# daooshee/ReReVST-Code

Measured on AMD Instinct MI355X. Metric: stylized frames/sec at 512x512, 1 style, higher is better.
Workload: dtype f32

## Files before the change

rerevst-code_amd/csrc/rerevst_hip.hip:

```cpp
#include <hip/hip_runtime.h>
#include <dlfcn.h>
#include <stddef.h>
#include <stdint.h>
#include <string.h>
#include <algorithm>
#include <cmath>
#include <thread>
#include <stdio.h>
#include <map>
#include <condition_variable>
#include <mutex>
#include <string>
#include <vector>

#include "../../include/rerevst_hip.h"
#include "conv_mfma.h"
#include "conv_wino.h"
#include "conv_wino_split.h"
#include "conv_f43.h"
#include "conv_thin.h"
#include "prep_kernels.h"
#include "mask_kernels.h"

namespace {

const int NORM_CH[11] = {512, 512, 256, 128, 64, 256, 256, 128, 128, 64, 64};
enum { N_DEC0 = 0, N_DEC1, N_DEC2, N_DEC3, N_DEC4, N_S4N1, N_S4N2, N_S3N1, N_S3N2, N_S2N1, N_S2N2 };
const int STYLE_CH[4] = {64, 128, 256, 512};
// ... 154 lines not shown
    unsigned launch_gen = 0;
    struct Feature { float* p; int H, W; uint8_t* u8; bool owned = true; };
    std::vector<Feature> features;
    std::vector<void*> feat_blocks;
    size_t feat_cap = (size_t)64 << 30, feat_bytes = 0;
    std::vector<float*> patches;
    int patch_h = 0, patch_w = 0, add_H = 0, add_W = 0;
    uint8_t* d_u8 = nullptr; size_t d_u8_cap = 0;
    float* d_outf = nullptr; size_t d_outf_cap = 0;
    double *stat_part = nullptr, *stat_part2 = nullptr, *stat_acc = nullptr;
    float *stat_mean = nullptr, *prep_cmean = nullptr;
    size_t ws_cap = (size_t)64 << 30;
    int last_groups = 0, last_group_size = 0; size_t last_ws_bytes = 0;
    PrepPlan prep;
    uint8_t* pend_u8 = nullptr; size_t pend_cap = 0; int pend_n = 0;
    InFmt pend_in = IN_BGR8;
    static constexpr int BLEND_W_RING = 4, BLEND_W_FLOATS = 64 * RRV_MAX_STYLES;
    struct BlendW { float* dev = nullptr; float* pin = nullptr; hipEvent_t ev[BLEND_W_RING] = {nullptr}; bool used[BLEND_W_RING] = {false}; unsigned gen = 0; } blend_w[2];
    const float* last_pre = nullptr; int last_pre_H = 0, last_pre_W = 0, last_pre_B = 0;
    struct StageBufs { uint8_t* in = nullptr; void* out = nullptr; size_t in_cap = 0, out_cap = 0; };
    struct HostStage {
        StageBufs dev, pin; hipEvent_t in_done = nullptr, k_done = nullptr, out_done = nullptr;
        float *mask = nullptr, *mask_pin = nullptr; size_t mask_cap = 0, mask_pin_cap = 0;
    } hstage[4];
    hipStream_t copy_in = nullptr, copy_out = nullptr;
    struct Ticket { long id = -1; void* out = nullptr; size_t out_bytes = 0; bool open = false; } tickets[4];
    long next_ticket = 0;
    int grid_share = 1;
    int f43_mode = 1;
    unsigned f43_layers = F43_DEFAULT_LAYERS;
    bool illcond = false;
    bool enc_p8_tables = false;
    int p8 = 3;
    bool f43_path = false;
    unsigned direct_layers = 0;
    int ms_group = 0;
    YuvSide yuv_in, yuv_out;
    int host_io = 0;
    int n_cus = 256;
    int debug = 0;
    int fail_alloc_in = 0;
    bool profiling = false;
    std::vector<ProfEntry> prof;
};

namespace {

#define HIPCHK(expr)                                                                              \
// ... 802 lines not shown
    RCHK(conv(h, c));
    const long npix = (long)B * (d.d.H + 2) * (d.d.W + 2);
    stamp(h, &d.d, B);
    return launch(h, "sum_parts", 0, 4.0 * 32 * (split + 1) * npix, [&] {
        const long nb = (npix * 8 + 255) / 256;
        hipLaunchKernelGGL(sum_parts_lrelu_k, dim3((unsigned)(nb < 4096 ? nb : 4096)), dim3(256), 0, h->stream, (const float*)t.p, d.d.p, split, npix);
    });
}

int filter_up(rrv_handle h, const Tens* cur, DecPlan& d, Tens* out, int f, int B) {
    const float* st = h->cur->active;
    ConvCall u{&d.d, out, &h->cur->fold_up[f], cur->H, cur->W}; u.B = B;
    if (h->state_images) { u.w_bstride = 512 * 32 * 16; u.par_bstride = RRV_STATE_FLOATS; }
    u.epi = E_RES | (f == 2 ? E_NORM2 : 0); u.res = cur;
    if (f == 2) { u.n2 = st + SL.norm[N_DEC1]; u.sty = st + SL.sty[3]; }
    return conv(h, u);
}

struct Win { int y0, x0, y1, x1; };

struct BlkDesc { const char* name; int cout, n1, n2, nada, sty; };
const BlkDesc BLKS[3] = {{"slice4", 256, N_S4N1, N_S4N2, N_DEC2, 2}, {"slice3", 128, N_S3N1, N_S3N2, N_DEC3, 1}, {"slice2", 64, N_S2N1, N_S2N2, N_DEC4, 0}};

int resblock_frame(rrv_handle h, int B, int k, const Tens& in, DecPlan& d, const Win* wa = nullptr, const Win* wo = nullptr) {
    const BlkDesc& b = BLKS[k];
    Tens &xs = d.xs[k], &a = d.a[k], &o = d.o[k], &qa = d.qa[k];
    const float* st = h->cur->active;
    const std::string p = std::string("Decoder.") + b.name;
    ConvCall c;
    const bool p8 = qa.p && use_f43(h, h->conv[p + ".conv2"], B, a.H, a.W, E_LRELU | E_NORM1 | E_RES_UPS | E_NORM2, false, 0, false) &&
                    !(wo && ((wo->y0 | wo->x0 | wo->y1 | wo->x1) & 31));
    Tens* a_in = p8 ? &qa : &a;
    c = ConvCall{&in, a_in, &h->conv[p + ".conv1"], a.H, a.W}; c.B = B; c.ups = true; c.epi = E_LRELU | E_NORM1; c.n1 = st + SL.norm[b.n1];
    c.sc_out = &xs; c.out_p8 = p8;
    if (h->state_images) c.par_bstride = RRV_STATE_FLOATS;
    if (wa) { c.wy0 = wa->y0; c.wx0 = wa->x0; c.wy1 = wa->y1; c.wx1 = wa->x1; }
    RCHK(conv(h, c));
    c = ConvCall{a_in, &o, &h->conv[p + ".conv2"], a.H, a.W}; c.B = B; c.in_p8 = p8;
    if (h->state_images) c.par_bstride = RRV_STATE_FLOATS;
    c.epi = E_LRELU | E_NORM1 | E_RES_UPS | E_NORM2; c.n1 = st + SL.norm[b.n2]; c.res = &xs; c.n2 = st + SL.norm[b.nada]; c.sty = st + SL.sty[b.sty];
    if (wo) { c.wy0 = wo->y0; c.wx0 = wo->x0; c.wy1 = wo->y1; c.wx1 = wo->x1; }
    RCHK(conv(h, c));
    return RRV_OK;
}

typedef void (*LastFn)(LastP);
LastFn last_kernel(OutFmt f) {
    if (yuv16_layout(f.yuv)) return conv_last_k<true, false, SP_PIXEL, true, true>;
    if (f.yuv) return conv_last_k<true, false, SP_PIXEL, true>;
    if (f.u8) return f.chw ? conv_last_k<true, true> : conv_last_k<true>;
    static const LastFn k[2][3] = {{conv_last_k<false>, conv_last_k<false, false, SP_UNIT>, conv_last_k<false, false, SP_NORM>},
                                   {conv_last_k<false, true>, conv_last_k<false, true, SP_UNIT>, conv_last_k<false, true, SP_NORM>}};
    return k[f.chw][f.space];
}

int run_last(rrv_handle h, const Tens& o2, int B, int H, int W, void* d_out, OutFmt fmt, float* pre, const PadCrop* pc, const Win* wl = nullptr) {
    LastP lp{o2.p, H, W, B, h->last_w, h->last_b, d_out, pre, (W + 15) / 16, (H + 15) / 16,
             pc ? pc->src_H : 0, pc ? pc->src_W : 0, pc ? pc->top : 0, pc ? pc->left : 0, 0, 0};
    if (fmt.yuv) {
        if (pc && ((pc->top | pc->left) & 1)) return fail(h, RRV_E_ARG, "conv_last: the YUV form needs an even crop origin");
        const YuvLaunch y = yuv_launch_params(h->yuv_out, false, yuv16_layout(fmt.yuv), fmt.yuv == RRV_LAY_P016);
        memcpy(lp.yuv_m, y.m, sizeof lp.yuv_m); lp.yuv_hi = y.hi; lp.yuv_shift = y.shift;
        lp.yuv_nv12 = fmt.yuv == RRV_LAY_NV12 || fmt.yuv == RRV_LAY_P016;
    }
    if (wl) { lp.ty0 = wl->y0 / 16; lp.tx0 = wl->x0 / 16; lp.tiles_y = (wl->y1 - wl->y0) / 16; lp.tiles_x = (wl->x1 - wl->x0) / 16; }
    h->last_pre = pre; h->last_pre_H = H; h->last_pre_W = W; h->last_pre_B = B;
    return launch(h, "conv_last", 2.0 * B * H * W * 576 * 3, (256.0 + (fmt.yuv ? 1.5 * yuv_sample_bytes(fmt) : 3.0 * out_elem(fmt))) * B * H * W, [&] {
        const unsigned tiles = (unsigned)(lp.tiles_x * lp.tiles_y * B), resident = (unsigned)h->n_cus * 4;
        hipLaunchKernelGGL(last_kernel(fmt), dim3(tiles < resident ? tiles : resident), dim3(256), 0, h->stream, lp);
    });
}

int transfer_device(rrv_handle h, int slot, const uint8_t* d_in, int B, int H, int W, void* d_out, const FrameIO& io, const float* feat = nullptr,
                    const float* const* feats = nullptr) {
    const PadCrop* const pc = io.pc;
    if (!h->finalized) return fail(h, RRV_E_WEIGHTS, "weights not finalized");
    const int Ho = H / 8 * 8, Wo = W / 8 * 8;
    RCHK(check_frame(h, H, W, "transfer"));
    if (h->active_src == -1) return fail(h, RRV_E_STATE, "state not computed: call compute() (or set_state) before transfer()");
    if (B < 1 || B > 64) return fail(h, RRV_E_ARG, "transfer: batch must be in 1..64");
    struct StreamScope { rrv_handle h; ~StreamScope() { h->stream = h->streams[0]; h->f43_path = false; } } scope{h};
    h->stream = h->streams[slot];
    if (slot < 2) h->set_images[slot] = 0;
    h->f43_path = true;
    if (h->caller_sync) {
        HIPCHK(hipEventRecord(h->slot_ev[slot], h->caller_stream));
        HIPCHK(hipStreamWaitEvent(h->stream, h->slot_ev[slot], 0));
    }
    EncPlan& e = pick_plan(h, h->enc_frame[slot], B, H, W);
    DecPlan& d = pick_plan(h, h->dec[slot], B, Ho, Wo);
    RCHK(enc_plan(h, e, B, H, W, true));
    RCHK(dec_plan(h, d, B, Ho, Wo));
    e.gen = d.gen = ++h->launch_gen;
    const float* st = h->cur->active;
    if (feats) {
        if (h->state_images != B) return fail(h, RRV_E_ARG, "transfer: per-image features need per-image state");
        for (int b = 0; b < B; ++b) {
// ... 18 lines not shown
        cur = &d.f[f];
    }
    Win wl{0, 0, 0, 0}, wo{0, 0, 0, 0}, wa{0, 0, 0, 0};
    const bool roi = pc != nullptr;
    if (roi) {
        auto grow = [&](const Win& w, int halo) {
            auto lo = [&](int v) { v -= halo; return v < 0 ? 0 : (v & ~15); };
            auto hi = [&](int v, int lim) { v = (v + halo + 15) & ~15; const int l = (lim + 15) & ~15; return v > l ? l : v; };
            return Win{lo(w.y0), lo(w.x0), hi(w.y1, Ho), hi(w.x1, Wo)};
        };
        const Win crop{pc->top, pc->left, pc->top + pc->src_H, pc->left + pc->src_W};
        wl = grow(crop, 0);
        wo = grow(crop, 1);
        if (use_f43(h, h->conv["Decoder.slice2.conv2"], B, Ho, Wo, E_LRELU | E_NORM1 | E_RES_UPS | E_NORM2, false, 0, false)) {
            const int lh = (Ho + 31) & ~31, lw = (Wo + 31) & ~31;
            wo = Win{wo.y0 & ~31, wo.x0 & ~31, (wo.y1 + 31) & ~31, (wo.x1 + 31) & ~31};
            if (wo.y1 > lh) wo.y1 = lh;
            if (wo.x1 > lw) wo.x1 = lw;
        }
        wa = grow(wo, 1);
    }
    for (int k = 0; k < 3; ++k) {
        const bool win = roi && k == 2;
        RCHK(resblock_frame(h, B, k, k ? d.o[k - 1] : d.f[2], d, win ? &wa : nullptr, win ? &wo : nullptr));
    }
    RCHK(run_last(h, d.o[2], B, Ho, Wo, d_out, io.out, d.pre, pc, roi ? &wl : nullptr));
    if (h->caller_sync) {
        HIPCHK(hipEventRecord(h->slot_ev[slot], h->stream));
        HIPCHK(hipStreamWaitEvent(h->caller_stream, h->slot_ev[slot], 0));
    }
    if (h->debug) RCHK(debug_verify(h, "transfer"));
    return RRV_OK;
}

enum { WALK_STOP = 1 };
template <class Stat, class Norm>
int unfused_blocks(rrv_handle h, int B, const Tens& x, Tens (&xs)[3], Tens (&a)[3], Tens (&o)[3], bool fused_sc, bool last_adain, Stat&& stat, Norm&& norm) {
    const Tens* in = &x;
    for (int k = 0; k < 3; ++k) {
        const BlkDesc& b = BLKS[k];
        const std::string p = std::string("Decoder.") + b.name;
        const int H2 = in->H * 2, W2 = in->W * 2;
        ConvCall c;
        c = ConvCall{in, &a[k], &h->conv[p + ".conv1"], H2, W2}; c.B = B; c.ups = true; c.epi = E_LRELU;
        if (fused_sc) c.sc_out = &xs[k];
        RCHK(conv(h, c));
        RCHK(stat(a[k], b.n1, 3 * k));
        RCHK(norm(a[k], a[k], b.n1, (const Tens*)nullptr, -1));
        c = ConvCall{&a[k], &o[k], &h->conv[p + ".conv2"], H2, W2}; c.B = B; c.epi = E_LRELU; RCHK(conv(h, c));
// ... 410 lines not shown
    return 0;
}

int rrv_create(int device, rrv_handle* out) {
    if (!out) return RRV_E_ARG;
    *out = nullptr;
    int n = 0;
    if (hipGetDeviceCount(&n) != hipSuccess || device < 0 || device >= n) return RRV_E_HIP;
    rrv_ctx* h = new rrv_ctx();
    h->dev = device;
    (void)rrv_yuv_input_matrix(RRV_YUV_BT601, 0, h->yuv_in.m8);
    (void)rrv_yuv_matrix(RRV_YUV_BT601, 0, h->yuv_out.m8);
    bool ok = hipSetDevice(device) == hipSuccess;
    for (int i = 0; ok && i < RRV_MAX_SLOTS; ++i) ok = hipStreamCreateWithFlags(&h->streams[i], hipStreamNonBlocking) == hipSuccess;
    if (!ok) {
        delete h;
        return RRV_E_HIP;
    }
    h->stream = h->streams[0];
    ok = ok && hipStreamCreateWithFlags(&h->copy_in, hipStreamNonBlocking) == hipSuccess && hipStreamCreateWithFlags(&h->copy_out, hipStreamNonBlocking) == hipSuccess;
    for (int i = 0; ok && i < RRV_MAX_SLOTS; ++i) ok = hipEventCreateWithFlags(&h->slot_ev[i], hipEventDisableTiming) == hipSuccess;
    for (auto& st : h->hstage)
        for (hipEvent_t* e : {&st.in_done, &st.k_done, &st.out_done}) ok = ok && hipEventCreateWithFlags(e, hipEventDisableTiming) == hipSuccess;
    for (const ConvKey& e : WINO_TABLE)
        if (ok && e.attr) ok = e.attr() == hipSuccess;
    for (const ConvKey& e : F43_TABLE)
        if (ok && e.attr) ok = e.attr() == hipSuccess;
    for (const F43LayKey& e : F43_LAY_TABLE)
        if (ok && e.attr) ok = e.attr() == hipSuccess;
    if (!ok) {
        delete h;
        return RRV_E_HIP;
    }
    {
        hipDeviceProp_t prop;
        if (hipGetDeviceProperties(&prop, device) == hipSuccess && prop.multiProcessorCount > 0) h->n_cus = prop.multiProcessorCount;
        const int masked = cu_mask_count(getenv("HSA_CU_MASK"), device, h->n_cus);
        if (masked > 0 && masked < h->n_cus) h->n_cus = masked;
        if (const char* e = getenv("RRV_CUS")) { const int n = atoi(e); if (n >= 1 && n <= 1024) h->n_cus = n; }
    }
    if (const char* e = getenv("RRV_F43_LAYERS")) h->f43_layers = (unsigned)strtoul(e, nullptr, 0);
    if (const char* e = getenv("RRV_DIRECT_LAYERS")) h->direct_layers = (unsigned)strtoul(e, nullptr, 0);
    if (const char* e = getenv("RRV_P8")) h->p8 = atoi(e) & 3;
    if (const char* e = getenv("RRV_F43")) h->f43_mode = atoi(e) < 0 ? 0 : (atoi(e) > 2 ? 2 : atoi(e));
    if (const char* e = getenv("RRV_DEBUG")) h->debug = atoi(e) < 0 ? 0 : (atoi(e) > 2 ? 2 : atoi(e));
    *out = h;
// ... 70 lines not shown
    for (int i = 0; i < 6; ++i) { if (h->fc_w[i]) (void)hipFree(h->fc_w[i]); if (h->fc_b[i]) (void)hipFree(h->fc_b[i]); }
    if (h->fold_tmp) (void)hipFree(h->fold_tmp);
    for (float* p : h->patches) (void)hipFree(p);
    for (auto& f : h->features) if (f.owned) { if (f.p) (void)hipFree(f.p); if (f.u8) (void)hipFree(f.u8); }
    for (void* b : h->feat_blocks) (void)hipFree(b);
    free_plans(h);
    for (StyleState& s : h->styles) { if (s.blob) (void)hipFree(s.blob); if (s.smean) (void)hipFree(s.smean); tfree(&s.map); }
    if (h->d_u8) (void)hipFree(h->d_u8);
    if (h->d_outf) (void)hipFree(h->d_outf);
    if (h->pend_u8) (void)hipFree(h->pend_u8);
    for (auto& bw : h->blend_w) {
        if (bw.dev) (void)hipFree(bw.dev);
        if (bw.pin) (void)hipHostFree(bw.pin);
        for (hipEvent_t e : bw.ev) if (e) (void)hipEventDestroy(e);
    }
    if (h->stat_part) (void)hipFree(h->stat_part);
    for (float* q : {h->first_w[0], h->first_w[1], h->first_b[0], h->first_b[1], h->first_wg}) if (q) (void)hipFree(q);
    for (auto& st : h->hstage) {
        stage_free(st.pin, true);
        stage_free(st.dev, false);
        if (st.mask) (void)hipFree(st.mask);
        if (st.mask_pin) (void)hipHostFree(st.mask_pin);
        for (hipEvent_t e : {st.in_done, st.k_done, st.out_done}) if (e) (void)hipEventDestroy(e);
    }
    if (h->copy_in) (void)hipStreamDestroy(h->copy_in);
    if (h->copy_out) (void)hipStreamDestroy(h->copy_out);
    for (ProfEntry& e : h->prof) { (void)hipEventDestroy(e.e0); (void)hipEventDestroy(e.e1); }
    for (int i = 0; i < RRV_MAX_SLOTS; ++i) { (void)hipStreamDestroy(h->streams[i]); if (h->slot_ev[i]) (void)hipEventDestroy(h->slot_ev[i]); }
    delete h;
    return RRV_OK;
}

const char* rrv_last_error(rrv_handle h) { return h ? h->err.c_str() : "null handle"; }

int rrv_load_weight(rrv_handle h, const char* key, const float* data, const int64_t* shape, int ndim) {
    if (!h || !key || !data || !shape || ndim < 1 || ndim > 4) return RRV_E_ARG;
    if (h->finalized) return fail(h, RRV_E_WEIGHTS, "weights already finalized");
    size_t n = 1;
    for (int i = 0; i < ndim; ++i) n *= (size_t)shape[i];
    h->hostw[key].assign(data, data + n);
    h->hostshape[key].assign(shape, shape + ndim);
    return RRV_OK;
}

int rrv_finalize_weights(rrv_handle h) {
    if (!h) return RRV_E_ARG;
    if (h->finalized) return RRV_OK;
// ... 462 lines not shown
    if (!bw.dev) RCHK(dalloc(h, &bw.dev, rrv_ctx::BLEND_W_FLOATS, false));
    if (!bw.pin) {
        void* p = nullptr;
        if (hipHostMalloc(&p, sizeof(float) * rrv_ctx::BLEND_W_RING * rrv_ctx::BLEND_W_FLOATS, hipHostMallocDefault) != hipSuccess) {
            (void)hipGetLastError();
            return fail(h, RRV_E_NOMEM, "blend weights: out of page-locked host memory");
        }
        bw.pin = (float*)p;
    }
    for (hipEvent_t& e : bw.ev)
        if (!e) HIPCHK(hipEventCreateWithFlags(&e, hipEventDisableTiming));
    const int g = (int)(bw.gen++ % rrv_ctx::BLEND_W_RING);
    if (bw.used[g]) HIPCHK(hipEventSynchronize(bw.ev[g]));
    float* const blk = bw.pin + (size_t)g * rrv_ctx::BLEND_W_FLOATS;
    memcpy(blk, wts, n * sizeof(float));
    HIPCHK(hipMemcpyAsync(bw.dev, blk, n * sizeof(float), hipMemcpyHostToDevice, h->streams[slot]));
    HIPCHK(hipEventRecord(bw.ev[g], h->streams[slot]));
    bw.used[g] = true;
    *d_w = bw.dev;
    return RRV_OK;
}


static int run_xfer(rrv_handle h, int slot, const void* d_in, void* d_out, const Xfer& x) {
    switch (x.model) {
    case Model::GLOBAL: RCHK(ensure_active(h)); break;
    case Model::FRAME:  if (h->active_src != -1) RCHK(sync_all(h)); break;
    case Model::BLEND:  if (h->active_src >= 0) RCHK(sync_all(h)); break;
    case Model::MASK:   break;
    }
    const bool bracket = h->caller_sync && x.model != Model::GLOBAL;
    if (bracket) {
        HIPCHK(hipEventRecord(h->slot_ev[slot], h->caller_stream));
        HIPCHK(hipStreamWaitEvent(h->streams[slot], h->slot_ev[slot], 0));
    }
    const float* d_w = x.wts;
    if (x.model == Model::BLEND && !x.w_dev) RCHK(stage_blend_weights(h, slot, x.wts, (size_t)x.B * x.ns, &d_w));
    const int KH = x.KH(), KW = x.KW(), G = x.model == Model::GLOBAL ? x.B : (int)rrv_ctx::MS_GROUP_MAX;
    const size_t fb = x.in_bytes(), fo = x.out_bytes();
    const PadCrop crop = x.pad_crop();
    const FrameIO io{x.in, x.fmt, x.pad ? &crop : nullptr};
    for (int b0 = 0; b0 < x.B; b0 += G) {
        const int cnt = x.B - b0 < G ? x.B - b0 : G;
        const uint8_t* const in = (const uint8_t*)d_in + (size_t)b0 * fb;
        void* const out = (char*)d_out + (size_t)b0 * fo;
        switch (x.model) {
        case Model::GLOBAL:
            RCHK(transfer_device(h, slot, in, cnt, KH, KW, out, io));
            break;
        case Model::FRAME:
            RCHK(frame_mode_device(h, slot, in, cnt, KH, KW, out, io));
            break;
        case Model::MASK:
            RCHK(mask_mode_device(h, slot, in, cnt, KH, KW, x.mask + (x.mask_images == 1 ? 0 : (size_t)b0 * x.mask_floats()), x.ns, x.mask_images == 1, out,
                                  io));
            break;
        case Model::BLEND: {
            SetScope scope{h, -2};
            h->stream = h->streams[slot];
            h->cur = &h->sets[rrv_ctx::MS_GROUP_MAX * slot];
            BlendDevP bp{};
            bp.n = x.ns; bp.out = h->cur->active; bp.count = RRV_STATE_FLOATS; bp.w = d_w + (size_t)b0 * x.ns;
            for (int s = 0; s < x.ns; ++s) bp.st[s] = h->styles[s].blob;
            hipLaunchKernelGGL(blend_states_dev_k, dim3((RRV_STATE_FLOATS + 255) / 256, cnt), dim3(256), 0, h->stream, bp);
            HIPCHK(hipGetLastError());
            h->active_src = -2;
            for (int f = 0; f < 3; ++f) RCHK(fold_filters(h, h->cur->active, f, cnt));
            h->state_images = cnt > 1 ? cnt : 0;
            RCHK(transfer_device(h, slot, in, cnt, KH, KW, out, io));
            h->set_images[slot] = cnt;
            break;
        }
        }
    }
    if (bracket) {
        HIPCHK(hipEventRecord(h->slot_ev[slot], h->streams[slot]));
        HIPCHK(hipStreamWaitEvent(h->caller_stream, h->slot_ev[slot], 0));
    }
    return RRV_OK;
}

static int next_frame_slot(rrv_handle h) { return next_device_slot(h) & 1; }
static int next_slot(rrv_handle h, const Xfer& x) { return x.model == Model::GLOBAL ? next_device_slot(h) : next_frame_slot(h); }

static int device_entry(rrv_handle h, const void* d_in, void* d_out, const Xfer& x) {
    if (!h || !d_in || !d_out) return RRV_E_ARG;
    HIPCHK(hipSetDevice(h->dev));
    RCHK(check_xfer(h, x));
    return run_xfer(h, next_slot(h, x), d_in, d_out, x);
}

int rrv_transfer_batch_device(rrv_handle h, const void* d_in, int B, int H, int W, void* d_out) {
// ... 211 lines not shown
    if (!call.owns_lock()) { memcpy(dst, src, bytes); return; }
    const size_t slice = ((bytes / nt) + 4095) & ~(size_t)4095;
    pool->run((char*)dst, (const char*)src, bytes, nt, slice);
}
static std::mutex g_pin_mu;
static std::map<const char*, size_t> g_pin_ranges;
static bool is_pinned(const void* ptr, size_t bytes) {
    {
        std::lock_guard<std::mutex> lk(g_pin_mu);
        auto it = g_pin_ranges.upper_bound((const char*)ptr);
        if (it != g_pin_ranges.begin()) {
            --it;
            if ((const char*)ptr + bytes <= it->first + it->second) return true;
        }
    }
    hipPointerAttribute_t a;
    for (const char* q : {(const char*)ptr, (const char*)ptr + (bytes ? bytes - 1 : 0)}) {
        if (hipPointerGetAttributes(&a, q) != hipSuccess) { (void)hipGetLastError(); return false; }
        if (a.type != hipMemoryTypeHost) return false;
    }
    return true;
}
static int retire_ticket(rrv_handle h, int set);
static int claim_staging(rrv_handle h) {
    for (int i = 0; i < HOST_SETS; ++i) RCHK(retire_ticket(h, i));
    RCHK(sync_all(h));
    h->next_slot = 0;
    return RRV_OK;
}
static int host_pipeline(rrv_handle h, const uint8_t* frames, void* out, const Xfer& x) {
    if (!h || !frames || !out) return RRV_E_ARG;
    HIPCHK(hipSetDevice(h->dev));
    RCHK(check_xfer(h, x, true));
    const int B = x.B;
    const float* const mask = x.mask;
    const int mask_images = x.mask_images;
    const size_t fb = x.in_bytes();
    const size_t fob = x.out_bytes();
    char* const outc = (char*)out;
    const int sub = x.model == Model::GLOBAL ? host_sub(B, x.KH(), x.KW()) : std::min(host_sub(B, x.KH(), x.KW()), (int)rrv_ctx::MS_GROUP_MAX);
    const size_t mfl = x.mask_floats();
    auto run = [&](int slot, int k, const void* d_in, int nb, void* d_out) -> int {
        Xfer part = x;
        part.B = nb;
        if (x.wts) part.wts = x.wts + (size_t)k * sub * x.ns;
        if (mask) { part.mask = h->hstage[k % HOST_SETS].mask; part.mask_images = mask_images == 1 ? 1 : nb; }
        return run_xfer(h, slot, d_in, d_out, part);
    };
    const bool in_pin = is_pinned(frames, (size_t)B * fb), out_pin = is_pinned(out, (size_t)B * fob);
    const size_t msub = (size_t)(mask_images == 1 ? 1 : sub) * mfl;
    const bool m_pin = mask && is_pinned(mask, (size_t)mask_images * mfl * sizeof(float));
    const bool host_in = !in_pin || (mask && !m_pin);
    RCHK(claim_staging(h));
    const int nchunk = (B + sub - 1) / sub;
    const int nsets = nchunk < HOST_SETS ? nchunk : HOST_SETS;
    const bool zin = h->host_io == 1 || h->host_io == 2, zout = h->host_io == 1 || h->host_io == 3;
    for (int i = 0; i < nsets; ++i) {
        RCHK(stage_reserve(h, i, zin ? 0 : (size_t)sub * fb, zout ? 0 : (size_t)sub * fob, false));
        RCHK(stage_reserve(h, i, in_pin ? 0 : (size_t)sub * fb, out_pin ? 0 : (size_t)sub * fob, true));
        if (!mask) continue;
        rrv_ctx::HostStage& st = h->hstage[i];
        RCHK(ensure_dev(h, st.mask, st.mask_cap, msub));
        if (!m_pin && st.mask_pin_cap < msub) {
            if (st.mask_pin) (void)hipHostFree(st.mask_pin);
            st.mask_pin = nullptr; st.mask_pin_cap = 0;
            if (hipHostMalloc((void**)&st.mask_pin, msub * sizeof(float), hipHostMallocDefault) != hipSuccess) {
                (void)hipGetLastError();
                st.mask_pin = nullptr;
                return fail(h, RRV_E_NOMEM, "staging: out of page-locked host memory");
            }
            st.mask_pin_cap = msub;
        }
    }
    auto count = [&](int k) { return (k + 1) * sub <= B ? sub : B - k * sub; };
    auto drain = [&](int k) -> int {
        auto& st = h->hstage[k % HOST_SETS];
        HIPCHK(hipEventSynchronize(st.out_done));
        if (!out_pin) host_copy(outc + (size_t)k * sub * fob, st.pin.out, (size_t)count(k) * fob);
        return RRV_OK;
    };
    int rc = RRV_OK;
    for (int k = 0; k < nchunk && rc == RRV_OK; ++k) {
        auto& st = h->hstage[k % HOST_SETS];
        const bool reuse = k >= HOST_SETS;
        if (reuse && (host_in || !out_pin)) rc = drain(k - HOST_SETS);
        if (rc != RRV_OK) break;
        const int nb = count(k);
        const uint8_t* src = frames + (size_t)k * sub * fb;
        if (!in_pin) { host_copy(st.pin.in, src, (size_t)nb * fb); src = st.pin.in; }
        const float* msrc = nullptr;
        size_t mbytes = 0;
        if (mask) {
            msrc = mask + (mask_images == 1 ? 0 : (size_t)k * sub * mfl);
            mbytes = (size_t)(mask_images == 1 ? 1 : nb) * mfl * sizeof(float);
            if (!m_pin) { host_copy(st.mask_pin, msrc, mbytes); msrc = st.mask_pin; }
        }
        const int slot = h->profiling ? 0 : (k & 1) % h->n_slots;
        hipStream_t cs = h->streams[slot];
        if (nchunk == 1 && h->host_io == 0) {
            HIPCHK(hipMemcpyAsync(st.dev.in, src, (size_t)nb * fb, hipMemcpyHostToDevice, cs));
            if (mask) HIPCHK(hipMemcpyAsync(st.mask, msrc, mbytes, hipMemcpyHostToDevice, cs));
            rc = run(slot, k, st.dev.in, nb, st.dev.out);
            if (rc != RRV_OK) break;
            HIPCHK(hipMemcpyAsync(out_pin ? out : st.pin.out, st.dev.out, (size_t)nb * fob, hipMemcpyDeviceToHost, cs));
            HIPCHK(hipStreamSynchronize(cs));
            if (!out_pin) host_copy(out, st.pin.out, (size_t)nb * fob);
            return RRV_OK;
        }
        const uint8_t* k_in = src;
        if (!zin || mask) {
            if (reuse) HIPCHK(hipStreamWaitEvent(h->copy_in, st.k_done, 0));
            if (!zin) {
                HIPCHK(hipMemcpyAsync(st.dev.in, src, (size_t)nb * fb, hipMemcpyHostToDevice, h->copy_in));
                k_in = st.dev.in;
            }
            if (mask) HIPCHK(hipMemcpyAsync(st.mask, msrc, mbytes, hipMemcpyHostToDevice, h->copy_in));
            HIPCHK(hipEventRecord(st.in_done, h->copy_in));
            HIPCHK(hipStreamWaitEvent(cs, st.in_done, 0));
        }
        void* const h_dst = out_pin ? outc + (size_t)k * sub * fob : st.pin.out;
        if (reuse) HIPCHK(hipStreamWaitEvent(cs, st.out_done, 0));
        void* const k_out = zout ? h_dst : st.dev.out;
        rc = run(slot, k, k_in, nb, k_out);
        if (rc != RRV_OK) break;
        if (!zin || mask) HIPCHK(hipEventRecord(st.k_done, cs));
        if (zout) { HIPCHK(hipEventRecord(st.out_done, cs)); continue; }
        if (zin && !mask) HIPCHK(hipEventRecord(st.k_done, cs));
        HIPCHK(hipStreamWaitEvent(h->copy_out, st.k_done, 0));
        HIPCHK(hipMemcpyAsync(h_dst, st.dev.out, (size_t)nb * fob, hipMemcpyDeviceToHost, h->copy_out));
        HIPCHK(hipEventRecord(st.out_done, h->copy_out));
    }
    if (rc != RRV_OK) { (void)sync_all(h); return rc; }
    const int first_open = (host_in || !out_pin) ? (nchunk - HOST_SETS < 0 ? 0 : nchunk - HOST_SETS) : 0;
    if (!host_in && out_pin) {
        if (zout) RCHK(sync_all(h));
        else HIPCHK(hipStreamSynchronize(h->copy_out));
    } else {
        for (int k = first_open; k < nchunk; ++k) RCHK(drain(k));
    }
    return RRV_OK;
}

int rrv_transfer(rrv_handle h, const uint8_t* frame, int H, int W, float* out) {
    return host_pipeline(h, frame, out, Xfer{Model::GLOBAL, 1, H, W, PLAIN, OUT_F32});
}
int rrv_transfer_u8(rrv_handle h, const uint8_t* frame, int H, int W, uint8_t* out) {
    return host_pipeline(h, frame, out, Xfer{Model::GLOBAL, 1, H, W, PLAIN, OUT_U8});
}

int rrv_transfer_batch(rrv_handle h, const uint8_t* frames, int B, int H, int W, float* out) {
    return host_pipeline(h, frames, out, Xfer{Model::GLOBAL, B, H, W, PLAIN, OUT_F32});
}
int rrv_transfer_batch_u8(rrv_handle h, const uint8_t* frames, int B, int H, int W, uint8_t* out) {
    return host_pipeline(h, frames, out, Xfer{Model::GLOBAL, B, H, W, PLAIN, OUT_U8});
}

int rrv_transfer_frames(rrv_handle h, const uint8_t* frames, int B, int H, int W, float* out) {
    return host_pipeline(h, frames, out, Xfer{Model::GLOBAL, B, H, W, PADDED, OUT_F32});
}
int rrv_transfer_frames_u8(rrv_handle h, const uint8_t* frames, int B, int H, int W, uint8_t* out) {
    return host_pipeline(h, frames, out, Xfer{Model::GLOBAL, B, H, W, PADDED, OUT_U8});
}
// ... 353 lines not shown
    if (!h || !wts || !out || ns < 1 || ns > RRV_MAX_STYLES) return RRV_E_ARG;
    if (feature_id < 0 || feature_id >= (int)h->features.size() || !(h->features[feature_id].p || h->features[feature_id].u8)) return RRV_E_ARG;
    HIPCHK(hipSetDevice(h->dev));
    RCHK(sync_all(h));
    h->next_slot = 0;
    const rrv_ctx::Feature& ft = h->features[feature_id];
    RCHK(blend_into_current(h, wts, ns));
    const size_t n = (size_t)(ft.H / 8 * 8) * (ft.W / 8 * 8) * 3;
    RCHK(ensure_dev(h, h->d_outf, h->d_outf_cap, out_floats(n, fmt)));
    RCHK(transfer_device(h, 0, ft.u8, 1, ft.H, ft.W, h->d_outf, FrameIO{IN_BGR8, fmt}, ft.p));
    HIPCHK(hipMemcpyAsync(out, h->d_outf, n * out_elem(fmt), hipMemcpyDeviceToHost, h->streams[0]));
    HIPCHK(hipStreamSynchronize(h->streams[0]));
    return RRV_OK;
}
int rrv_transfer_features(rrv_handle h, int feature_id, const float* wts, int ns, float* out) {
    return transfer_features(h, feature_id, wts, ns, out, OUT_F32);
}
int rrv_transfer_features_u8(rrv_handle h, int feature_id, const float* wts, int ns, uint8_t* out) {
    return transfer_features(h, feature_id, wts, ns, out, OUT_U8);
}

static int transfer_features_batch(rrv_handle h, const int* ids, const float* wts, int n, int ns, void* out, OutFmt fmt) {
    if (!h || !ids || !wts || !out || n < 1 || ns < 1 || ns > RRV_MAX_STYLES) return RRV_E_ARG;
    HIPCHK(hipSetDevice(h->dev));
    for (int i = 0; i < n; ++i)
        if (ids[i] < 0 || ids[i] >= (int)h->features.size() || !(h->features[ids[i]].p || h->features[ids[i]].u8)) return fail(h, RRV_E_ARG, "transfer: unknown feature id");
    for (int s = 0; s < ns; ++s)
        if (!h->styles[s].computed) return fail(h, RRV_E_STATE, "blend: state not computed for every style");
    const int H = h->features[ids[0]].H, W = h->features[ids[0]].W;
    for (int i = 1; i < n; ++i)
        if (h->features[ids[i]].H != H || h->features[ids[i]].W != W) return fail(h, RRV_E_ARG, "transfer: features of one call must share their size");
    RCHK(claim_staging(h));
    const size_t npx = (size_t)(H / 8 * 8) * (W / 8 * 8) * 3 * out_elem(fmt);
    const FrameIO io{IN_BGR8, fmt};
    char* const outc = (char*)out;
    const bool out_pin = is_pinned(out, (size_t)n * npx);
    int G = h->ms_group;
    if (G == 0) {
        const long s = HOST_SUB_PIXELS / ((long)H * W);
        G = s < 1 ? 1 : s > rrv_ctx::MS_GROUP_MAX ? rrv_ctx::MS_GROUP_MAX : (int)s;
    }
    if (G > n) G = n;
    struct Group { int first, count; };
    std::vector<Group> groups;
    for (int i = 0; i < n;) {
        if (!h->features[ids[i]].p) { groups.push_back({i, 1}); ++i; continue; }
        int c = 0;
        while (c < G && i + c < n && h->features[ids[i + c]].p) ++c;
        groups.push_back({i, c});
        i += c;
    }
    const int ngroups = (int)groups.size();
    const int nslots = (h->profiling || h->n_slots < 2 || ngroups < 2) ? 1 : 2;
    for (int i = 0; i < nslots; ++i) {
        RCHK(stage_reserve(h, i, 0, (size_t)G * npx, false));
        RCHK(stage_reserve(h, i, 0, out_pin ? 0 : (size_t)G * npx, true));
    }
    SetScope scope{h, -2};
    auto drain = [&](int k) -> int {
        auto& st = h->hstage[k % nslots];
        HIPCHK(hipEventSynchronize(st.out_done));
        if (!out_pin) host_copy(outc + (size_t)groups[k].first * npx, st.pin.out, (size_t)groups[k].count * npx);
        return RRV_OK;
    };
    for (int k = 0; k < ngroups; ++k) {
        const int slot = k % nslots, first = groups[k].first, cnt = groups[k].count;
        auto& st = h->hstage[slot];
        if (k >= nslots) {
            if (!out_pin) RCHK(drain(k - nslots));
            HIPCHK(hipStreamWaitEvent(h->streams[slot], st.out_done, 0));
        }
        h->stream = h->streams[slot];
        const float* fp[rrv_ctx::MS_GROUP_MAX] = {};
        h->cur = &h->sets[rrv_ctx::MS_GROUP_MAX * slot];
        {
            static_assert(rrv_ctx::MS_GROUP_MAX <= 16, "BlendManyP::w holds sixteen images");
            BlendManyP bp{};
            bp.n = ns; bp.out = h->cur->active; bp.count = RRV_STATE_FLOATS;
            for (int s = 0; s < ns; ++s) bp.st[s] = h->styles[s].blob;
            for (int g = 0; g < cnt; ++g) {
                for (int s = 0; s < ns; ++s) bp.w[g][s] = wts[(size_t)(first + g) * ns + s];
                fp[g] = h->features[ids[first + g]].p;
            }
            hipLaunchKernelGGL(blend_states_k, dim3((RRV_STATE_FLOATS + 255) / 256, cnt), dim3(256), 0, h->stream, bp);
            HIPCHK(hipGetLastError());
            for (int f = 0; f < 3; ++f) RCHK(fold_filters(h, h->cur->active, f, cnt));
        }
        h->active_src = -2;
        if (fp[0] && cnt == 1) {
            RCHK(transfer_device(h, slot, nullptr, 1, H, W, st.dev.out, io, fp[0]));
        } else if (fp[0]) {
            h->state_images = cnt;
            const int rc = transfer_device(h, slot, nullptr, cnt, H, W, st.dev.out, io, nullptr, fp);
            h->state_images = 0;
            RCHK(rc);
        } else {
            RCHK(transfer_device(h, slot, h->features[ids[first]].u8, 1, H, W, st.dev.out, io));
        }
        h->set_images[slot] = cnt;
        HIPCHK(hipEventRecord(st.k_done, h->streams[slot]));
        HIPCHK(hipStreamWaitEvent(h->copy_out, st.k_done, 0));
        HIPCHK(hipMemcpyAsync(out_pin ? (void*)(outc + (size_t)first * npx) : st.pin.out, st.dev.out, (size_t)cnt * npx, hipMemcpyDeviceToHost, h->copy_out));
        HIPCHK(hipEventRecord(st.out_done, h->copy_out));
    }
    if (out_pin) HIPCHK(hipStreamSynchronize(h->copy_out));
    else for (int k = (ngroups - nslots < 0 ? 0 : ngroups - nslots); k < ngroups; ++k) RCHK(drain(k));
    return RRV_OK;
}
int rrv_transfer_features_batch(rrv_handle h, const int* ids, const float* wts, int n, int ns, float* out) {
    return transfer_features_batch(h, ids, wts, n, ns, out, OUT_F32);
}
int rrv_transfer_features_batch_u8(rrv_handle h, const int* ids, const float* wts, int n, int ns, uint8_t* out) {
    return transfer_features_batch(h, ids, wts, n, ns, out, OUT_U8);
}

int rrv_release_features(rrv_handle h) {
    if (!h) return RRV_E_ARG;
    HIPCHK(hipSetDevice(h->dev));
    RCHK(sync_all(h));
    for (auto& f : h->features) if (f.owned) { if (f.p) (void)hipFree(f.p); if (f.u8) (void)hipFree(f.u8); }
    for (void* b : h->feat_blocks) (void)hipFree(b);
    h->feat_blocks.clear();
    h->features.clear();
    h->feat_bytes = 0;
    return RRV_OK;
}

static int transfer_frame_mode(rrv_handle h, const uint8_t* frame, int H, int W, void* out, OutFmt fmt) {
    if (!h || !frame || !out) return RRV_E_ARG;
// ... 224 lines not shown
```

Measured before the change: 858.2.

## Order chunk tails across slots and stream final chunk's output in pieces

In the host pipeline with multiple chunks and slots, the last resblock's second conv of each chunk now waits for the previous chunk's kernels to finish. This phases the two slot streams so one chunk's tail finishes earlier instead of both contending for the GPU at once. The final chunk runs its last conv in frame-range pieces, each followed by an immediate device-to-host copy, so the trailing D2H overlaps the remaining compute. Env knobs and an optional event timeline print are added for diagnosis. The added dependency can reduce concurrency between slots, and extra launches and events add overhead.

```diff
diff --git a/rerevst-code_amd/csrc/rerevst_hip.hip b/rerevst-code_amd/csrc/rerevst_hip.hip
--- a/rerevst-code_amd/csrc/rerevst_hip.hip
+++ b/rerevst-code_amd/csrc/rerevst_hip.hip
@@ -4,6 +4,7 @@
 #include <stdint.h>
 #include <string.h>
 #include <algorithm>
+#include <chrono>
 #include <cmath>
 #include <thread>
 #include <stdio.h>
@@ -204,8 +205,17 @@
     struct HostStage {
         StageBufs dev, pin; hipEvent_t in_done = nullptr, k_done = nullptr, out_done = nullptr;
         float *mask = nullptr, *mask_pin = nullptr; size_t mask_cap = 0, mask_pin_cap = 0;
+        static constexpr int PIECES_MAX = 16;
+        hipEvent_t piece_ev[PIECES_MAX] = {nullptr};
     } hstage[4];
     hipStream_t copy_in = nullptr, copy_out = nullptr;
+    bool host_phase = true;
+    long host_piece_px = 2L * 640 * 640;
+    struct Timeline {
+        static constexpr int N = 64;
+        bool on = false;
+        hipEvent_t entry = nullptr, first = nullptr, k_end[N] = {nullptr}, d_end[N] = {nullptr};
+    } tl;
     struct Ticket { long id = -1; void* out = nullptr; size_t out_bytes = 0; bool open = false; } tickets[4];
     long next_ticket = 0;
     int grid_share = 1;
@@ -1054,7 +1064,7 @@
 struct BlkDesc { const char* name; int cout, n1, n2, nada, sty; };
 const BlkDesc BLKS[3] = {{"slice4", 256, N_S4N1, N_S4N2, N_DEC2, 2}, {"slice3", 128, N_S3N1, N_S3N2, N_DEC3, 1}, {"slice2", 64, N_S2N1, N_S2N2, N_DEC4, 0}};
 
-int resblock_frame(rrv_handle h, int B, int k, const Tens& in, DecPlan& d, const Win* wa = nullptr, const Win* wo = nullptr) {
+int resblock_frame(rrv_handle h, int B, int k, const Tens& in, DecPlan& d, const Win* wa = nullptr, const Win* wo = nullptr, hipEvent_t mid_wait = nullptr) {
     const BlkDesc& b = BLKS[k];
     Tens &xs = d.xs[k], &a = d.a[k], &o = d.o[k], &qa = d.qa[k];
     const float* st = h->cur->active;
@@ -1068,6 +1078,7 @@
     if (h->state_images) c.par_bstride = RRV_STATE_FLOATS;
     if (wa) { c.wy0 = wa->y0; c.wx0 = wa->x0; c.wy1 = wa->y1; c.wx1 = wa->x1; }
     RCHK(conv(h, c));
+    if (mid_wait) HIPCHK(hipStreamWaitEvent(h->stream, mid_wait, 0));
     c = ConvCall{a_in, &o, &h->conv[p + ".conv2"], a.H, a.W}; c.B = B; c.in_p8 = p8;
     if (h->state_images) c.par_bstride = RRV_STATE_FLOATS;
     c.epi = E_LRELU | E_NORM1 | E_RES_UPS | E_NORM2; c.n1 = st + SL.norm[b.n2]; c.res = &xs; c.n2 = st + SL.norm[b.nada]; c.sty = st + SL.sty[b.sty];
@@ -1086,9 +1097,18 @@
     return k[f.chw][f.space];
 }
 
-int run_last(rrv_handle h, const Tens& o2, int B, int H, int W, void* d_out, OutFmt fmt, float* pre, const PadCrop* pc, const Win* wl = nullptr) {
+struct FrameRange { int first, count; size_t out_bytes; };
+int run_last(rrv_handle h, const Tens& o2, int B, int H, int W, void* d_out, OutFmt fmt, float* pre, const PadCrop* pc, const Win* wl = nullptr,
+             const FrameRange* fr = nullptr) {
     LastP lp{o2.p, H, W, B, h->last_w, h->last_b, d_out, pre, (W + 15) / 16, (H + 15) / 16,
              pc ? pc->src_H : 0, pc ? pc->src_W : 0, pc ? pc->top : 0, pc ? pc->left : 0, 0, 0};
+    if (fr) {
+        lp.in += (size_t)fr->first * (size_t)(H + 2) * (size_t)(W + 2) * 64;
+        lp.out_img = (char*)d_out + (size_t)fr->first * fr->out_bytes;
+        if (pre) lp.out_pre = pre + (size_t)fr->first * H * W * 3;
+        lp.B = fr->count;
+    }
+    const int LB = lp.B;
     if (fmt.yuv) {
         if (pc && ((pc->top | pc->left) & 1)) return fail(h, RRV_E_ARG, "conv_last: the YUV form needs an even crop origin");
         const YuvLaunch y = yuv_launch_params(h->yuv_out, false, yuv16_layout(fmt.yuv), fmt.yuv == RRV_LAY_P016);
@@ -1097,14 +1117,19 @@
     }
     if (wl) { lp.ty0 = wl->y0 / 16; lp.tx0 = wl->x0 / 16; lp.tiles_y = (wl->y1 - wl->y0) / 16; lp.tiles_x = (wl->x1 - wl->x0) / 16; }
     h->last_pre = pre; h->last_pre_H = H; h->last_pre_W = W; h->last_pre_B = B;
-    return launch(h, "conv_last", 2.0 * B * H * W * 576 * 3, (256.0 + (fmt.yuv ? 1.5 * yuv_sample_bytes(fmt) : 3.0 * out_elem(fmt))) * B * H * W, [&] {
-        const unsigned tiles = (unsigned)(lp.tiles_x * lp.tiles_y * B), resident = (unsigned)h->n_cus * 4;
+    return launch(h, "conv_last", 2.0 * LB * H * W * 576 * 3, (256.0 + (fmt.yuv ? 1.5 * yuv_sample_bytes(fmt) : 3.0 * out_elem(fmt))) * LB * H * W, [&] {
+        const unsigned tiles = (unsigned)(lp.tiles_x * lp.tiles_y * LB), resident = (unsigned)h->n_cus * 4;
         hipLaunchKernelGGL(last_kernel(fmt), dim3(tiles < resident ? tiles : resident), dim3(256), 0, h->stream, lp);
     });
 }
 
+struct SeqHook {
+    hipEvent_t tail_wait = nullptr;
+    int piece = 0; char* h_dst = nullptr; size_t frame_bytes = 0; hipStream_t copy = nullptr; hipEvent_t* ev = nullptr;
+};
+
 int transfer_device(rrv_handle h, int slot, const uint8_t* d_in, int B, int H, int W, void* d_out, const FrameIO& io, const float* feat = nullptr,
-                    const float* const* feats = nullptr) {
+                    const float* const* feats = nullptr, const SeqHook* hk = nullptr) {
     const PadCrop* const pc = io.pc;
     if (!h->finalized) return fail(h, RRV_E_WEIGHTS, "weights not finalized");
     const int Ho = H / 8 * 8, Wo = W / 8 * 8;
@@ -1169,9 +1194,21 @@
     }
     for (int k = 0; k < 3; ++k) {
         const bool win = roi && k == 2;
-        RCHK(resblock_frame(h, B, k, k ? d.o[k - 1] : d.f[2], d, win ? &wa : nullptr, win ? &wo : nullptr));
-    }
-    RCHK(run_last(h, d.o[2], B, Ho, Wo, d_out, io.out, d.pre, pc, roi ? &wl : nullptr));
+        RCHK(resblock_frame(h, B, k, k ? d.o[k - 1] : d.f[2], d, win ? &wa : nullptr, win ? &wo : nullptr, hk && k == 2 ? hk->tail_wait : nullptr));
+    }
+    if (hk && hk->piece > 0 && hk->piece < B) {
+        int i = 0;
+        for (int b0 = 0; b0 < B; b0 += hk->piece, ++i) {
+            const FrameRange fr{b0, B - b0 < hk->piece ? B - b0 : hk->piece, hk->frame_bytes};
+            RCHK(run_last(h, d.o[2], B, Ho, Wo, d_out, io.out, d.pre, pc, roi ? &wl : nullptr, &fr));
+            const size_t off = (size_t)b0 * hk->frame_bytes;
+            HIPCHK(hipEventRecord(hk->ev[i], h->stream));
+            HIPCHK(hipStreamWaitEvent(hk->copy, hk->ev[i], 0));
+            HIPCHK(hipMemcpyAsync(hk->h_dst + off, (const char*)d_out + off, (size_t)fr.count * hk->frame_bytes, hipMemcpyDeviceToHost, hk->copy));
+        }
+    } else {
+        RCHK(run_last(h, d.o[2], B, Ho, Wo, d_out, io.out, d.pre, pc, roi ? &wl : nullptr));
+    }
     if (h->caller_sync) {
         HIPCHK(hipEventRecord(h->slot_ev[slot], h->stream));
         HIPCHK(hipStreamWaitEvent(h->caller_stream, h->slot_ev[slot], 0));
@@ -1628,6 +1665,15 @@
     for (int i = 0; ok && i < RRV_MAX_SLOTS; ++i) ok = hipEventCreateWithFlags(&h->slot_ev[i], hipEventDisableTiming) == hipSuccess;
     for (auto& st : h->hstage)
         for (hipEvent_t* e : {&st.in_done, &st.k_done, &st.out_done}) ok = ok && hipEventCreateWithFlags(e, hipEventDisableTiming) == hipSuccess;
+    for (auto& st : h->hstage)
+        for (hipEvent_t& e : st.piece_ev) ok = ok && hipEventCreateWithFlags(&e, hipEventDisableTiming) == hipSuccess;
+    if (const char* e = getenv("RRV_HOST_PHASE")) h->host_phase = atoi(e) != 0;
+    if (const char* e = getenv("RRV_HOST_PIECE")) { const long n = atol(e); h->host_piece_px = (n < 0 ? 0 : n > 64 ? 64 : n) * 640L * 640L; }
+    if (const char* e = getenv("RRV_TIMELINE")) h->tl.on = atoi(e) != 0;
+    if (h->tl.on) {
+        ok = ok && hipEventCreate(&h->tl.entry) == hipSuccess && hipEventCreate(&h->tl.first) == hipSuccess;
+        for (int i = 0; i < rrv_ctx::Timeline::N; ++i) ok = ok && hipEventCreate(&h->tl.k_end[i]) == hipSuccess && hipEventCreate(&h->tl.d_end[i]) == hipSuccess;
+    }
     for (const ConvKey& e : WINO_TABLE)
         if (ok && e.attr) ok = e.attr() == hipSuccess;
     for (const ConvKey& e : F43_TABLE)
@@ -1744,7 +1790,11 @@
         if (st.mask) (void)hipFree(st.mask);
         if (st.mask_pin) (void)hipHostFree(st.mask_pin);
         for (hipEvent_t e : {st.in_done, st.k_done, st.out_done}) if (e) (void)hipEventDestroy(e);
-    }
+        for (hipEvent_t e : st.piece_ev) if (e) (void)hipEventDestroy(e);
+    }
+    for (hipEvent_t e : {h->tl.entry, h->tl.first}) if (e) (void)hipEventDestroy(e);
+    for (int i = 0; i < rrv_ctx::Timeline::N; ++i)
+        for (hipEvent_t e : {h->tl.k_end[i], h->tl.d_end[i]}) if (e) (void)hipEventDestroy(e);
     if (h->copy_in) (void)hipStreamDestroy(h->copy_in);
     if (h->copy_out) (void)hipStreamDestroy(h->copy_out);
     for (ProfEntry& e : h->prof) { (void)hipEventDestroy(e.e0); (void)hipEventDestroy(e.e1); }
@@ -2253,7 +2303,7 @@
 }
 
 
-static int run_xfer(rrv_handle h, int slot, const void* d_in, void* d_out, const Xfer& x) {
+static int run_xfer(rrv_handle h, int slot, const void* d_in, void* d_out, const Xfer& x, const SeqHook* hk = nullptr) {
     switch (x.model) {
     case Model::GLOBAL: RCHK(ensure_active(h)); break;
     case Model::FRAME:  if (h->active_src != -1) RCHK(sync_all(h)); break;
@@ -2277,7 +2327,7 @@
         void* const out = (char*)d_out + (size_t)b0 * fo;
         switch (x.model) {
         case Model::GLOBAL:
-            RCHK(transfer_device(h, slot, in, cnt, KH, KW, out, io));
+            RCHK(transfer_device(h, slot, in, cnt, KH, KW, out, io, nullptr, nullptr, hk));
             break;
         case Model::FRAME:
             RCHK(frame_mode_device(h, slot, in, cnt, KH, KW, out, io));
@@ -2298,7 +2348,7 @@
             h->active_src = -2;
             for (int f = 0; f < 3; ++f) RCHK(fold_filters(h, h->cur->active, f, cnt));
             h->state_images = cnt > 1 ? cnt : 0;
-            RCHK(transfer_device(h, slot, in, cnt, KH, KW, out, io));
+            RCHK(transfer_device(h, slot, in, cnt, KH, KW, out, io, nullptr, nullptr, hk));
             h->set_images[slot] = cnt;
             break;
         }
@@ -2556,6 +2606,28 @@
     return true;
 }
 static int retire_ticket(rrv_handle h, int set);
+static int timeline_print(rrv_handle h, const char* who, int frames, int H, int W, int n, double setup_ms, double wall_ms) {
+    auto& tl = h->tl;
+    auto at = [&](hipEvent_t e) { float ms = -1.f; if (hipEventElapsedTime(&ms, tl.entry, e) != hipSuccess) { (void)hipGetLastError(); ms = -1.f; } return ms; };
+    std::string line;
+    char b[96];
+    snprintf(b, sizeof b, "rrv_timeline %s frames=%d size=%dx%d subs=%d", who, frames, H, W, n); line += b;
+    snprintf(b, sizeof b, " setup=%.3f wall=%.3f first_kernel=%.3f k_end=", setup_ms, wall_ms, at(tl.first)); line += b;
+    for (int k = 0; k < n; ++k) { snprintf(b, sizeof b, "%s%.3f", k ? "," : "", at(tl.k_end[k])); line += b; }
+    line += " d2h_end=";
+    for (int k = 0; k < n; ++k) { snprintf(b, sizeof b, "%s%.3f", k ? "," : "", at(tl.d_end[k])); line += b; }
+    fprintf(stderr, "%s\n", line.c_str());
+    return RRV_OK;
+}
+static double host_ms_since(std::chrono::steady_clock::time_point t0) { return std::chrono::duration<double, std::milli>(std::chrono::steady_clock::now() - t0).count(); }
+static int tail_piece(rrv_handle h, int nb, int H, int W) {
+    if (h->host_piece_px <= 0) return 0;
+    long p = h->host_piece_px / ((long)H * W);
+    const long least = (nb + rrv_ctx::HostStage::PIECES_MAX - 1) / rrv_ctx::HostStage::PIECES_MAX;
+    if (p < least) p = least;
+    if (p < 1) p = 1;
+    return p < nb ? (int)p : 0;
+}
 static int claim_staging(rrv_handle h) {
     for (int i = 0; i < HOST_SETS; ++i) RCHK(retire_ticket(h, i));
     RCHK(sync_all(h));
@@ -2564,6 +2636,7 @@
 }
 static int host_pipeline(rrv_handle h, const uint8_t* frames, void* out, const Xfer& x) {
     if (!h || !frames || !out) return RRV_E_ARG;
+    const auto t_entry = std::chrono::steady_clock::now();
     HIPCHK(hipSetDevice(h->dev));
     RCHK(check_xfer(h, x, true));
     const int B = x.B;
@@ -2574,12 +2647,12 @@
     char* const outc = (char*)out;
     const int sub = x.model == Model::GLOBAL ? host_sub(B, x.KH(), x.KW()) : std::min(host_sub(B, x.KH(), x.KW()), (int)rrv_ctx::MS_GROUP_MAX);
     const size_t mfl = x.mask_floats();
-    auto run = [&](int slot, int k, const void* d_in, int nb, void* d_out) -> int {
+    auto run = [&](int slot, int k, const void* d_in, int nb, void* d_out, const SeqHook* hk) -> int {
         Xfer part = x;
         part.B = nb;
         if (x.wts) part.wts = x.wts + (size_t)k * sub * x.ns;
         if (mask) { part.mask = h->hstage[k % HOST_SETS].mask; part.mask_images = mask_images == 1 ? 1 : nb; }
-        return run_xfer(h, slot, d_in, d_out, part);
+        return run_xfer(h, slot, d_in, d_out, part, hk);
     };
     const bool in_pin = is_pinned(frames, (size_t)B * fb), out_pin = is_pinned(out, (size_t)B * fob);
     const size_t msub = (size_t)(mask_images == 1 ? 1 : sub) * mfl;
@@ -2589,6 +2662,11 @@
     const int nchunk = (B + sub - 1) / sub;
     const int nsets = nchunk < HOST_SETS ? nchunk : HOST_SETS;
     const bool zin = h->host_io == 1 || h->host_io == 2, zout = h->host_io == 1 || h->host_io == 3;
+    const bool ordered = nchunk > 1 && h->n_slots > 1 && !h->profiling && !h->debug && !h->caller_sync && h->host_io == 0 &&
+                         (x.model == Model::GLOBAL || x.model == Model::BLEND);
+    const bool tl_on = h->tl.on && nchunk > 1 && nchunk <= rrv_ctx::Timeline::N && h->host_io == 0;
+    double tl_setup = 0;
+    if (tl_on) { tl_setup = host_ms_since(t_entry); HIPCHK(hipEventRecord(h->tl.entry, h->streams[0])); }
     for (int i = 0; i < nsets; ++i) {
         RCHK(stage_reserve(h, i, zin ? 0 : (size_t)sub * fb, zout ? 0 : (size_t)sub * fob, false));
         RCHK(stage_reserve(h, i, in_pin ? 0 : (size_t)sub * fb, out_pin ? 0 : (size_t)sub * fob, true));
@@ -2634,7 +2712,7 @@
         if (nchunk == 1 && h->host_io == 0) {
             HIPCHK(hipMemcpyAsync(st.dev.in, src, (size_t)nb * fb, hipMemcpyHostToDevice, cs));
             if (mask) HIPCHK(hipMemcpyAsync(st.mask, msrc, mbytes, hipMemcpyHostToDevice, cs));
-            rc = run(slot, k, st.dev.in, nb, st.dev.out);
+            rc = run(slot, k, st.dev.in, nb, st.dev.out, nullptr);
             if (rc != RRV_OK) break;
             HIPCHK(hipMemcpyAsync(out_pin ? out : st.pin.out, st.dev.out, (size_t)nb * fob, hipMemcpyDeviceToHost, cs));
             HIPCHK(hipStreamSynchronize(cs));
@@ -2655,14 +2733,27 @@
         void* const h_dst = out_pin ? outc + (size_t)k * sub * fob : st.pin.out;
         if (reuse) HIPCHK(hipStreamWaitEvent(cs, st.out_done, 0));
         void* const k_out = zout ? h_dst : st.dev.out;
-        rc = run(slot, k, k_in, nb, k_out);
+        SeqHook hk;
+        if (ordered) {
+            if (h->host_phase && k > 0) hk.tail_wait = h->hstage[(k - 1) % HOST_SETS].k_done;
+            if (k == nchunk - 1) {
+                hk.piece = tail_piece(h, nb, x.KH(), x.KW());
+                hk.h_dst = (char*)h_dst; hk.frame_bytes = fob; hk.copy = h->copy_out; hk.ev = st.piece_ev;
+            }
+        }
+        if (tl_on && k == 0) HIPCHK(hipEventRecord(h->tl.first, cs));
+        rc = run(slot, k, k_in, nb, k_out, ordered ? &hk : nullptr);
         if (rc != RRV_OK) break;
+        if (tl_on) HIPCHK(hipEventRecord(h->tl.k_end[k], cs));
         if (!zin || mask) HIPCHK(hipEventRecord(st.k_done, cs));
         if (zout) { HIPCHK(hipEventRecord(st.out_done, cs)); continue; }
         if (zin && !mask) HIPCHK(hipEventRecord(st.k_done, cs));
-        HIPCHK(hipStreamWaitEvent(h->copy_out, st.k_done, 0));
-        HIPCHK(hipMemcpyAsync(h_dst, st.dev.out, (size_t)nb * fob, hipMemcpyDeviceToHost, h->copy_out));
+        if (hk.piece == 0) {
+            HIPCHK(hipStreamWaitEvent(h->copy_out, st.k_done, 0));
+            HIPCHK(hipMemcpyAsync(h_dst, st.dev.out, (size_t)nb * fob, hipMemcpyDeviceToHost, h->copy_out));
+        }
         HIPCHK(hipEventRecord(st.out_done, h->copy_out));
+        if (tl_on) HIPCHK(hipEventRecord(h->tl.d_end[k], h->copy_out));
     }
     if (rc != RRV_OK) { (void)sync_all(h); return rc; }
     const int first_open = (host_in || !out_pin) ? (nchunk - HOST_SETS < 0 ? 0 : nchunk - HOST_SETS) : 0;
@@ -2672,6 +2763,7 @@
     } else {
         for (int k = first_open; k < nchunk; ++k) RCHK(drain(k));
     }
+    if (tl_on) RCHK(timeline_print(h, "host_pipeline", B, x.KH(), x.KW(), nchunk, tl_setup, host_ms_since(t_entry)));
     return RRV_OK;
 }
 
@@ -3071,6 +3163,7 @@
 
 static int transfer_features_batch(rrv_handle h, const int* ids, const float* wts, int n, int ns, void* out, OutFmt fmt) {
     if (!h || !ids || !wts || !out || n < 1 || ns < 1 || ns > RRV_MAX_STYLES) return RRV_E_ARG;
+    const auto t_entry = std::chrono::steady_clock::now();
     HIPCHK(hipSetDevice(h->dev));
     for (int i = 0; i < n; ++i)
         if (ids[i] < 0 || ids[i] >= (int)h->features.size() || !(h->features[ids[i]].p || h->features[ids[i]].u8)) return fail(h, RRV_E_ARG, "transfer: unknown feature id");
@@ -3106,6 +3199,9 @@
         RCHK(stage_reserve(h, i, 0, out_pin ? 0 : (size_t)G * npx, true));
     }
     SetScope scope{h, -2};
+    const bool tl_on = h->tl.on && ngroups > 1 && ngroups <= rrv_ctx::Timeline::N;
+    double tl_setup = 0;
+    if (tl_on) { tl_setup = host_ms_since(t_entry); HIPCHK(hipEventRecord(h->tl.entry, h->streams[0])); }
     auto drain = [&](int k) -> int {
         auto& st = h->hstage[k % nslots];
         HIPCHK(hipEventSynchronize(st.out_done));
@@ -3136,6 +3232,8 @@
             for (int f = 0; f < 3; ++f) RCHK(fold_filters(h, h->cur->active, f, cnt));
         }
         h->active_src = -2;
+        void* const h_dst = out_pin ? (void*)(outc + (size_t)first * npx) : st.pin.out;
+        if (tl_on && k == 0) HIPCHK(hipEventRecord(h->tl.first, h->streams[slot]));
         if (fp[0] && cnt == 1) {
             RCHK(transfer_device(h, slot, nullptr, 1, H, W, st.dev.out, io, fp[0]));
         } else if (fp[0]) {
@@ -3147,13 +3245,16 @@
             RCHK(transfer_device(h, slot, h->features[ids[first]].u8, 1, H, W, st.dev.out, io));
         }
         h->set_images[slot] = cnt;
+        if (tl_on) HIPCHK(hipEventRecord(h->tl.k_end[k], h->streams[slot]));
         HIPCHK(hipEventRecord(st.k_done, h->streams[slot]));
         HIPCHK(hipStreamWaitEvent(h->copy_out, st.k_done, 0));
-        HIPCHK(hipMemcpyAsync(out_pin ? (void*)(outc + (size_t)first * npx) : st.pin.out, st.dev.out, (size_t)cnt * npx, hipMemcpyDeviceToHost, h->copy_out));
+        HIPCHK(hipMemcpyAsync(h_dst, st.dev.out, (size_t)cnt * npx, hipMemcpyDeviceToHost, h->copy_out));
         HIPCHK(hipEventRecord(st.out_done, h->copy_out));
+        if (tl_on) HIPCHK(hipEventRecord(h->tl.d_end[k], h->copy_out));
     }
     if (out_pin) HIPCHK(hipStreamSynchronize(h->copy_out));
     else for (int k = (ngroups - nslots < 0 ? 0 : ngroups - nslots); k < ngroups; ++k) RCHK(drain(k));
+    if (tl_on) RCHK(timeline_print(h, "transfer_features_batch", n, H, W, ngroups, tl_setup, host_ms_since(t_entry)));
     return RRV_OK;
 }
 int rrv_transfer_features_batch(rrv_handle h, const int* ids, const float* wts, int n, int ns, float* out) {
```

After: 868.3 (median of 6 runs). 1.2% higher.
